# y00njaekim/CMU-11785-IDL-1.58bit-ASR

Hardware: AMD Instinct MI355X
Metric: mel-frames/sec (Conformer-S 1.58-bit train step) (higher is better)
Workload: dtype fp32; 1 GPU; conformer-s-1.58bit-train-step; global_batch=32, execution=hip-graph, per_gpu_batch=32, frames=1000, d_model=144, blocks=16, d_ff=576, heads=4, vocab=5004, parallelism=dp1, passes=teacher 2-bit + student 1-bit + SP, conv_pointwise=fp32 (reference)

## Files before the change

cmu-11785-idl-1.58bit-asr_amd/csrc/capi.hip:

```cpp
#include <algorithm>
#include <vector>

#include "../../include/onebit_hip.h"
#include "ob_launch.h"
#include <stdint.h>

using namespace ob;

namespace {

constexpr int kAbiVersion = 4;

inline hipStream_t as_stream(void* s) { return reinterpret_cast<hipStream_t>(s); }

inline bool aligned4(const void* p) { return (reinterpret_cast<uintptr_t>(p) & 3) == 0; }

inline int check_bits(int bits) { return (bits == 1 || bits == 2) ? OB_OK : OB_ERR_BITWIDTH; }

inline int launched() {
  const hipError_t e = hipGetLastError();
  return e == hipSuccess ? OB_OK : OB_ERR_HIP;
}

inline size_t align_up(size_t x) { return (x + 255) & ~size_t(255); }

struct DwWorkspace {
  size_t part, part_db, apart, total;
};

DwWorkspace dw_layout(int64_t P, int64_t M, int64_t N, int64_t K, int64_t G = 1) {
  const DwPlan p = plan_dw_passes(P, M, G * N, K);
  DwWorkspace w;
  w.part = align_up(sizeof(float) * (size_t)p.chunks * (size_t)N * (size_t)K);
  w.part_db = align_up(sizeof(float) * (size_t)p.chunks * (size_t)N);
  const int64_t napart = std::max<int64_t>(ste_reduce_blocks(N * K + N),
                                           p.tiles_n * p.tiles_k * p.chunks);
  w.apart = align_up(16 + sizeof(float) * (size_t)napart);
  w.total = w.part + w.part_db + w.apart;
  return w;
}

}

extern "C" {

int ob_abi_version(void) { return kAbiVersion; }

const char* ob_status_string(int status) {
  switch (status) {
    case OB_OK: return "ok";
    case OB_ERR_NULL: return "null pointer argument";
    case OB_ERR_SHAPE: return "invalid shape";
    case OB_ERR_BITWIDTH: return "bitwidth must be one of {1,2,32}";
    case OB_ERR_WORKSPACE: return "workspace too small";
    case OB_ERR_ALIGN: return "pointer not 4-byte aligned";
    case OB_ERR_HIP: return "HIP launch error";
    default: return "unknown status";
  }
}

int ob_quant_pack(const float* W, const float* alpha, int alpha_raw, int bits, int64_t N,
                  int64_t K, uint32_t* codes, uint32_t* codes_t, void* stream) {
  if (int st = check_bits(bits)) return st;
  if (N < 0 || K < 0) return OB_ERR_SHAPE;
// ... 310 lines not shown
      (nln > 1 && (!a16(ln_y1) || !a16(ln_w1) || !a16(ln_b1))) || !aligned4(bias) ||
      !aligned4(lens) || !aligned4(ln_mean0) || !aligned4(ln_rstd0) || !aligned4(ln_mean1) ||
      !aligned4(ln_rstd1))
    return OB_ERR_ALIGN;
  TgemmEpi ep{};
  ep.mode = kEpiResidual;
  ep.R = R;
  ep.rscale = rscale;
  ep.lens = reinterpret_cast<const int*>(lens);
  ep.T = (int)T;
  ep.p_drop = p_drop;
  ep.rng = rng;
  ep.rng_off = (uint64_t)rng_offset;
  ep.nln = nln;
  ep.lng[0] = ln_w0;
  ep.lnb[0] = ln_b0;
  ep.lneps[0] = eps0;
  ep.lny[0] = ln_y0;
  ep.lnmean[0] = ln_mean0;
  ep.lnrstd[0] = ln_rstd0;
  ep.lng[1] = ln_w1;
  ep.lnb[1] = ln_b1;
  ep.lneps[1] = eps1;
  ep.lny[1] = ln_y1;
  ep.lnmean[1] = ln_mean1;
  ep.lnrstd[1] = ln_rstd1;
  launch_ternary_gemm_passes(X, (int)P, M, K, codes2, pass_bits ? codes1 : codes2,
                             reinterpret_cast<const int*>(pass_bits), N, alpha, alpha_raw, bias, Y,
                             as_stream(stream), &ep);
  return launched();
}

int ob_bitlinear_bwd_dx_swish_drop(const float* dY, int64_t P, int64_t M, int64_t N,
                                   const uint32_t* codes2_t, const uint32_t* codes1_t,
                                   const int32_t* pass_bits, const float* alpha, int alpha_raw,
                                   int64_t K, const float* pre, float p_drop, const uint64_t* rng,
                                   int64_t rng_offset, float* dPre, void* stream) {
  if (int st = fused_gemm_check(dY, P, M, N, codes2_t, codes1_t, pass_bits, alpha, K, dPre, p_drop,
                                rng))
    return st;
  if (M * K > 0 && !pre) return OB_ERR_NULL;
  if (!aligned4(pre)) return OB_ERR_ALIGN;
  TgemmEpi ep{};
  ep.mode = kEpiSwishDropBwd;
  ep.R = pre;
  ep.p_drop = p_drop;
  ep.rng = rng;
  ep.rng_off = (uint64_t)rng_offset;
  launch_ternary_gemm_passes(dY, (int)P, M, N, codes2_t, pass_bits ? codes1_t : codes2_t,
                             reinterpret_cast<const int*>(pass_bits), K, alpha, alpha_raw, nullptr,
                             dPre, as_stream(stream), &ep);
  return launched();
}

int ob_drop_scale_bwd(const float* dOut, int64_t rows, int64_t N, float rscale, float p_drop,
                      const uint64_t* rng, int64_t rng_offset, const int32_t* lens, int64_t T,
                      float* dY, void* stream) {
  if (rows < 0 || N < 0 || !(p_drop >= 0.0f && p_drop < 1.0f)) return OB_ERR_SHAPE;
  if (lens && (T < 1 || T > 0x7fffffff || rows % T)) return OB_ERR_SHAPE;
  if ((rows * N > 0 && (!dOut || !dY)) || (p_drop > 0.0f && !rng)) return OB_ERR_NULL;
  if ((reinterpret_cast<uintptr_t>(dOut) & 15) || (reinterpret_cast<uintptr_t>(dY) & 15) ||
      !aligned4(lens))
    return OB_ERR_ALIGN;
  launch_drop_scale_bwd(dOut, rows, N, rscale, p_drop, rng, (uint64_t)rng_offset,
                        reinterpret_cast<const int*>(lens), (int)T, dY, as_stream(stream));
  return launched();
}

int ob_residual_drop_fwd(const float* R, const float* Y, int64_t rows, int64_t N, float rscale,
                         float p_drop, const uint64_t* rng, int64_t rng_offset,
                         const int32_t* lens, int64_t T, float* out, void* stream) {
  if (rows < 0 || N < 0 || !(p_drop >= 0.0f && p_drop < 1.0f)) return OB_ERR_SHAPE;
  if (lens && (T < 1 || T > 0x7fffffff || rows % T)) return OB_ERR_SHAPE;
  if ((rows * N > 0 && (!R || !Y || !out)) || (p_drop > 0.0f && !rng)) return OB_ERR_NULL;
  if (!aligned4(R) || !aligned4(Y) || !aligned4(out) || !aligned4(lens)) return OB_ERR_ALIGN;
  launch_residual_drop_fwd(R, Y, rows, N, rscale, p_drop, rng, (uint64_t)rng_offset,
                           reinterpret_cast<const int*>(lens), (int)T, out, as_stream(stream));
  return launched();
}

int ob_bias_relu_fwd(float* y, const float* bias, int64_t B, int64_t C, int64_t hw,
                     void* stream) {
  if (B < 0 || C < 0 || hw < 0) return OB_ERR_SHAPE;
  if (B * C * hw > 0 && (!y || !bias)) return OB_ERR_NULL;
  if (!aligned4(y) || !aligned4(bias)) return OB_ERR_ALIGN;
  if (hw % 4 == 0 && (reinterpret_cast<uintptr_t>(y) & 15)) return OB_ERR_ALIGN;
  launch_bias_relu_fwd(y, bias, B, C, hw, as_stream(stream));
  return launched();
}

size_t ob_relu_bias_bwd_workspace(int64_t B, int64_t C) {
  return (B < 0 || C < 0) ? 0 : relu_bias_bwd_workspace(B, C);
}

int ob_relu_bias_bwd(const float* g, const float* y, int64_t B, int64_t C, int64_t hw,
                     float* gout, float* dbias, void* ws, size_t ws_bytes, void* stream) {
  if (B < 0 || C < 0 || hw < 0 || B * C > 0x7fffffff) return OB_ERR_SHAPE;
  if (B * C * hw > 0 && (!g || !y || !gout)) return OB_ERR_NULL;
  if (B * C > 0 && !ws) return OB_ERR_NULL;
  if (ws_bytes < relu_bias_bwd_workspace(B, C)) return OB_ERR_WORKSPACE;
  if (!aligned4(g) || !aligned4(y) || !aligned4(gout) || !aligned4(dbias)) return OB_ERR_ALIGN;
  launch_relu_bias_bwd(g, y, B, C, hw, gout, dbias, ws, as_stream(stream));
  return launched();
}

size_t ob_colsum_workspace(int64_t N) { return N < 0 ? 0 : colsum_workspace(N); }
// ... 1177 lines not shown
```

cmu-11785-idl-1.58bit-asr_amd/csrc/ob_launch.h:

```cpp
#pragma once

#include <hip/hip_runtime.h>
#include <stddef.h>
#include <stdint.h>

#include "../../include/onebit_hip.h"

namespace ob {

inline int64_t ceil_div(int64_t a, int64_t b) { return (a + b - 1) / b; }

void launch_quant_pack(const float* W, const float* alpha, int alpha_raw, int bits,
                       const int* bits_dev, int64_t N, int64_t K, uint32_t* codes,
                       uint32_t* codes_t, hipStream_t s);
int64_t quant_pack_item_blocks(int64_t N, int64_t K);
int64_t quant_pack_item_blocks16(int64_t N, int64_t K);
void launch_quant_pack_group(const ob_pack_item* items_dev, int n_items, int64_t total_blocks,
                             hipStream_t s);
void launch_quant_dequant(const float* W, const float* alpha, int alpha_raw, int bits, int64_t n,
                          float* W_hat, hipStream_t s);

int64_t ste_reduce_blocks(int64_t total);
void launch_ste_reduce(const float* part, int chunks, int64_t nk, const float* part_db,
                       int64_t n_db, const float* W, const float* alpha, int alpha_raw, int bits,
                       const int* bits_dev, float* dW, float* db, float* apart, uint32_t* ticket,
                       float* dalpha, hipStream_t s);
constexpr int kMaxPasses = 4;
void launch_ste_reduce_passes(const float* part, int P, int cpp, int64_t nk, const float* part_db,
                              int64_t n_db, const float* W, const float* alpha, int alpha_raw,
                              const int* pass_bits, float* dW, float* db, float* apart,
                              uint32_t* ticket, float* dalpha, hipStream_t s);

bool launch_ternary_gemm_signacc(const float* A, int64_t M, int64_t K, const uint32_t* codes,
                                 int64_t N, const float* alpha, int alpha_raw, const float* bias,
                                 float* C, hipStream_t s);
void launch_ternary_gemm(const float* A, int64_t M, int64_t K, const uint32_t* codes, int64_t N,
                         const float* alpha, int alpha_raw, const float* bias, float* C,
                         hipStream_t s);

struct TgemmEpi;
void launch_ternary_gemm_passes(const float* A, int P, int64_t M, int64_t K,
                                const uint32_t* codes, const uint32_t* codes1,
                                const int* pass_bits, int64_t N, const float* alpha,
                                int alpha_raw, const float* bias, float* C, hipStream_t s,
                                const TgemmEpi* ep = nullptr);
bool launch_ternary_gemm_passes_group(const float* A, int P, int64_t M, int64_t K, int G,
                                      const uint32_t* const* codes,
                                      const uint32_t* const* codes1, const int* pass_bits,
                                      int64_t N, const float* const* alpha, int alpha_raw,
                                      const float* const* bias, float* const* C, hipStream_t s);
bool launch_ternary_dx_sum(int G, const float* const* dY, int P, int64_t M, int64_t N,
                           const uint32_t* const* codes_t, const uint32_t* const* codes_t1,
                           const int* pass_bits, const float* const* alpha, int alpha_raw,
                           int64_t K, float* dX, hipStream_t s);

enum { kEpiNone = 0, kEpiSwishDrop = 1, kEpiResidual = 2, kEpiSwishDropBwd = 3 };
struct TgemmEpi {
  int mode;
  const float* R;
  float* C2;
  float rscale;
  const int* lens;
  int T;
  float p_drop;
  const uint64_t* rng;
  uint64_t rng_off;
  int nln;
  const float* lng[2];
  const float* lnb[2];
  float lneps[2];
  float* lny[2];
  float* lnmean[2];
  float* lnrstd[2];
};
bool ternary_residual_ln_supported(int64_t K, int64_t N, int alpha_raw);

void launch_residual_drop_fwd(const float* R, const float* Y, int64_t rows, int64_t N,
                              float rscale, float p_drop, const uint64_t* rng, uint64_t rng_off,
                              const int* lens, int T, float* out, hipStream_t s);

void launch_bias_relu_fwd(float* y, const float* bias, int64_t B, int64_t C, int64_t hw,
                          hipStream_t s);
size_t relu_bias_bwd_workspace(int64_t B, int64_t C);
void launch_relu_bias_bwd(const float* g, const float* y, int64_t B, int64_t C, int64_t hw,
                          float* gout, float* dbias, void* ws, hipStream_t s);
void launch_zero_words(void* p, int64_t n_words, hipStream_t s);
size_t colsum_workspace(int64_t N);
void launch_colsum(const float* x, int64_t rows, int64_t N, float* out, void* ws, hipStream_t s);

bool decattn_supported(int64_t Lq, int64_t Lk, int64_t dh);
void launch_decattn_fwd(const float* q, int64_t sq, const float* k, int64_t sk, const float* v,
                        int64_t sv, const uint8_t* kmask, int causal, int64_t B, int64_t H,
                        int64_t Lq, int64_t Lk, int64_t dh, float p_drop, const uint64_t* rng,
                        uint64_t rng_off, float* probs, float* ctx, hipStream_t s);
void launch_decattn_bwd(const float* dctx, const float* ctxo, const float* q, int64_t sq,
                        const float* k, int64_t sk, const float* v, int64_t sv, int64_t B, int64_t H, int64_t Lq, int64_t Lk,
                        int64_t dh, float p_drop, float* probs, float* dq, int64_t gq,
                        float* dk, int64_t gk, float* dv, int64_t gv, hipStream_t s);
// ... 293 lines not shown
```

cmu-11785-idl-1.58bit-asr_amd/csrc/tgemm.hip:

```cpp
#include <cstdlib>

#include "ob_drop.h"
#include "ob_fp.h"
#include "ob_ln.h"
#include "ob_launch.h"
#include "ob_quant.h"

namespace ob {

namespace {

typedef float f32x4 __attribute__((ext_vector_type(4)));
typedef __bf16 bf16x8 __attribute__((ext_vector_type(8)));
typedef uint32_t u32x4 __attribute__((ext_vector_type(4)));

constexpr int kThreads = 256;
constexpr int kRows = 64;
constexpr size_t kMaxLds = 80 * 1024;
constexpr int kTargetBlocks = 512;
constexpr int kTargetBlocksLongK = 256;
constexpr int kByteWaves = 8;
constexpr int kBPad = 16;
constexpr int kBytePad = 8;

__device__ __forceinline__ void code_bytes(uint32_t word, u32x4& out) {
#pragma unroll
  for (int q = 0; q < 4; ++q) {
    uint32_t x = (word >> (8 * q)) & 0xFFu;
    x = (x | (x << 6) | (x << 12) | (x << 18)) & 0x03030303u;
    const uint32_t lo = x & 0x01010101u, hi = x & 0x02020202u;
    out[q] = ((lo << 6) - lo) | (hi << 6);
  }
}

__device__ __forceinline__ bf16x8 bytes_bf16x8(uint32_t d0, uint32_t d1) {
  u32x4 o;
  o[0] = __builtin_amdgcn_perm(d1, d0, 0x010C000Cu);
  o[1] = __builtin_amdgcn_perm(d1, d0, 0x030C020Cu);
  o[2] = __builtin_amdgcn_perm(d1, d0, 0x050C040Cu);
  o[3] = __builtin_amdgcn_perm(d1, d0, 0x070C060Cu);
  return __builtin_bit_cast(bf16x8, o);
}

#ifdef OB_TGEMM_STAMPS
__device__ uint64_t g_tg_stamps[32768];
__device__ uint64_t g_tg_rt[16384];
#define TG_DECL                                                              \
  uint64_t tg_t = __builtin_amdgcn_s_memtime(), tg_rt0 = __builtin_amdgcn_s_memrealtime(), \
           tg_acc[4] = {0, 0, 0, 0};
#define TG_STAMP(k)                                       \
  do {                                                    \
    const uint64_t tg_n = __builtin_amdgcn_s_memtime();   \
// ... 568 lines not shown
            } else {
              epi_store4<EPI>(ep, dkey, C + orow * N + col, rowbase + orow, col, N, y, rvalid[it],
                              rpre[it]);
            }
          }
        }
        asm volatile("s_waitcnt lgkmcnt(0)" ::: "memory");
        __builtin_amdgcn_sched_barrier(0);
      }
      TG_STAMP(2);
      continue;
    }
    if constexpr (!VEC_EPI) {

    constexpr bool kHasR = EPI == kEpiResidual || EPI == kEpiSwishDropBwd;
    constexpr int kPre = 2;
    float rv[NT][4];
    auto load_r = [&](int t) {
      const int col = min(n0 + 16 * t + r, N - 1);
#pragma unroll
      for (int reg = 0; reg < 4; ++reg) {
        const int64_t orow = min(m0 + 4 * g + reg, M - 1);
        rv[t][reg] = ep.R[(rowbase + orow) * N + col];
      }
    };
    if constexpr (kHasR) {
#pragma unroll
      for (int t = 0; t < kPre && t < NT; ++t) load_r(t);
    }
#pragma unroll
    for (int t = 0; t < NT; ++t) {
      if constexpr (kHasR) {
        if (t + kPre < NT) load_r(t + kPre);
        __builtin_amdgcn_sched_barrier(0);
      }
      const int col = n0 + 16 * t + r;
      if (col >= N) continue;
#pragma unroll
      for (int reg = 0; reg < 4; ++reg) {
        const int64_t orow = m0 + 4 * g + reg;
        if (orow >= M) continue;
        const float y = fmaf(a_eff, acc[t][reg], bcol[t]);
        if constexpr (EPI == kEpiNone) {
          C[orow * N + col] = y;
          if (EPI == kEpiSwishDrop) ep.C2[(rowbase + orow) * N + col] = y;
        } else {
          epi_store<EPI>(ep, dkey, C + orow * N + col, rowbase + orow, col, N, y, rv[t][reg]);
        }
      }
      if constexpr (EPI != kEpiNone) __builtin_amdgcn_sched_barrier(0);
    }
    TG_STAMP(2);
    }
  }
  TG_WRITE
}

constexpr int kF32NT = 3;

__global__ __launch_bounds__(kThreads) void tgemm_f32_kernel(
    const float* __restrict__ A, int64_t M, int64_t K, const uint32_t* __restrict__ codes,
    int64_t KW, int64_t N, const float* __restrict__ alpha, int alpha_raw,
    const float* __restrict__ bias, float* __restrict__ C, const uint32_t* __restrict__ codes1,
    const int* __restrict__ pass_bits, EpiArgs ep) {
  const int64_t rowbase = pass_bits ? (int64_t)blockIdx.z * M : 0;
  if (pass_bits) {
    const int p = blockIdx.z;
    if (pass_bits[p] == 1) codes = codes1;
    A += (int64_t)p * M * K;
    C += (int64_t)p * M * N;
  }
  const int lane = threadIdx.x & 63;
  const int wave = threadIdx.x >> 6;
  const int r = lane & 15;
  const int g = lane >> 4;
  const int64_t m0 = (int64_t)blockIdx.x * kRows + wave * 16;
  const int64_t n0 = (int64_t)blockIdx.y * (16 * kF32NT);
  const int64_t row = m0 + r < M ? m0 + r : M - 1;
  const float* arow = A + row * K;
  f32x4 acc[kF32NT];
#pragma unroll
  for (int t = 0; t < kF32NT; ++t) acc[t] = f32x4{0.f, 0.f, 0.f, 0.f};
  for (int64_t kc = 0; kc < K; kc += 16) {
    float xa[4];
#pragma unroll
    for (int e = 0; e < 4; ++e) {
      const int64_t k = kc + 4 * g + e;
      xa[e] = arow[k < K ? k : K - 1];
    }
#pragma unroll
    for (int t = 0; t < kF32NT; ++t) {
      const int64_t n = n0 + 16 * t + r;
      if (alpha_raw >= 2) {
        const uint16_t* Wb = reinterpret_cast<const uint16_t*>(codes);
#pragma unroll
        for (int e = 0; e < 4; ++e) {
          const int64_t k = kc + 4 * g + e;
          const float w = (n < N && k < K) ? __uint_as_float((uint32_t)Wb[n * K + k] << 16) : 0.0f;
          acc[t] = __builtin_amdgcn_mfma_f32_16x16x4f32(xa[e], w, acc[t], 0, 0, 0);
        }
        continue;
      }
      const uint32_t word = codes[(n < N ? n : N - 1) * KW + (kc >> 4)];
      const uint32_t byte = (n < N) ? (word >> (8 * g)) : 0u;
#pragma unroll
      for (int e = 0; e < 4; ++e)
// ... 73 lines not shown
  const size_t lds = epi_stage_off(NT, kpad, byte) +
                     (byte && ep.mode == kEpiResidual
                          ? (size_t)wv * 16 * (16 * NT + 4) * sizeof(float) + 4 * 16 * NT * sizeof(float)
                          : epi_stage_bytes(NT, wv));
  const int KW = (int)ceil_div(K, 16);
  const bool vec = (N % 4 == 0) && aligned16(C) && (ep.mode != kEpiSwishDrop || aligned16(ep.C2)) &&
                   ((ep.mode != kEpiResidual && ep.mode != kEpiSwishDropBwd) || aligned16(ep.R));
#define OB_TGEMM_E(NCH, E)                                                                     \
  if (vec)                                                                                    \
    hipLaunchKernelGGL((tgemm_bf16x3_kernel<NT, NCH, E, true>), grid, dim3(kThreads), lds, s,  \
                       A, M, (int)K, codes, KW, (int)N, n_ct, n16, rgroups, alpha, alpha_raw,  \
                       bias, C, codes1, pass_bits, ep);                                         \
  else                                                                                        \
    hipLaunchKernelGGL((tgemm_bf16x3_kernel<NT, NCH, E, false>), grid, dim3(kThreads), lds, s, \
                       A, M, (int)K, codes, KW, (int)N, n_ct, n16, rgroups, alpha, alpha_raw,  \
                       bias, C, codes1, pass_bits, ep)
  if constexpr (NT == 9) {
    if (byte) {
#define OB_TGEMM_B(E)                                                                            \
  if (vec)                                                                                      \
    hipLaunchKernelGGL((tgemm_bf16x3_kernel<9, 18, E, true, true, 1, kByteWaves>), grid,         \
                       dim3(64 * kByteWaves), lds, s,                                            \
                       A, M, (int)K, codes, KW, (int)N, n_ct, n16, rgroups, alpha, alpha_raw,    \
                       bias, C, codes1, pass_bits, ep);                                           \
  else                                                                                          \
    hipLaunchKernelGGL((tgemm_bf16x3_kernel<9, 18, E, false, true, 1, kByteWaves>), grid,        \
                       dim3(64 * kByteWaves), lds,                                               \
                       s, A, M, (int)K, codes, KW, (int)N, n_ct, n16, rgroups, alpha, alpha_raw, \
                       bias, C, codes1, pass_bits, ep)
      if (ep.mode == kEpiResidual) OB_TGEMM_B(kEpiResidual);
      else OB_TGEMM_B(kEpiNone);
#undef OB_TGEMM_B
      return;
    }
  }
#define OB_TGEMM(NCH)                                                   \
  switch (ep.mode) {                                                    \
    case kEpiSwishDrop: OB_TGEMM_E(NCH, kEpiSwishDrop); break;          \
    case kEpiResidual: OB_TGEMM_E(NCH, kEpiResidual); break;            \
    case kEpiSwishDropBwd: OB_TGEMM_E(NCH, kEpiSwishDropBwd); break;    \
    default: OB_TGEMM_E(NCH, kEpiNone); break;                          \
  }
  switch ((K + 31) / 32) {
    case 2: OB_TGEMM(2); break;
    case 5: OB_TGEMM(5); break;
    case 8: OB_TGEMM(8); break;
    case 18: OB_TGEMM(18); break;
    default: OB_TGEMM(0); break;
  }
#undef OB_TGEMM
#undef OB_TGEMM_E
}

}

void launch_ternary_gemm_passes(const float* A, int P, int64_t M, int64_t K,
                                const uint32_t* codes, const uint32_t* codes1,
                                const int* pass_bits, int64_t N, const float* alpha,
                                int alpha_raw, const float* bias, float* C, hipStream_t s,
                                const TgemmEpi* epi) {
  if (M == 0 || N == 0 || P == 0) return;
  EpiArgs ep{};
  ep.glayers = 1;
  ep.mode = kEpiNone;
  if (epi && epi->mode != kEpiNone) {
    ep.mode = epi->mode;
    ep.R = epi->R;
    ep.C2 = epi->C2;
    ep.rscale = epi->rscale;
    ep.lens = epi->lens;
    ep.T = epi->T > 0 ? epi->T : 1;
    ep.dc = make_drop(epi->p_drop);
    ep.rng = epi->rng;
    ep.rng_off = epi->rng_off;
    ep.nln = epi->nln;
    for (int i = 0; i < 2; ++i) {
      ep.lng[i] = epi->lng[i];
      ep.lnb[i] = epi->lnb[i];
      ep.lneps[i] = epi->lneps[i];
      ep.lny[i] = epi->lny[i];
      ep.lnmean[i] = epi->lnmean[i];
      ep.lnrstd[i] = epi->lnrstd[i];
    }
  }
  const bool vec = (K % 4 == 0) && K >= 4 && ((reinterpret_cast<uintptr_t>(A) & 15) == 0);
  const int nt = vec && !use_f32_gemm() ? pick_nt(N, K, ep.mode) : 0;
  if (nt > 0 && (K + 31) / 32 == 18 && N % 144 == 0 && alpha_raw < 2 &&
      (ep.mode == kEpiNone || ep.mode == kEpiResidual)) {
    launch_bf16x3<9>(A, M, K, codes, N, alpha, alpha_raw, bias, C, codes1, pass_bits, P, ep, s, true);
    return;
  }
#define OB_NT(V)                                                                            \
  case V:                                                                                   \
    launch_bf16x3<V>(A, M, K, codes, N, alpha, alpha_raw, bias, C, codes1, pass_bits, P, ep, s); \
    return;
  switch (nt) {
    OB_NT(12)
    OB_NT(9)
    OB_NT(6)
    OB_NT(4)
    OB_NT(3)
    OB_NT(2)
    OB_NT(1)
    default: break;
  }
#undef OB_NT
  const dim3 grid((unsigned)ceil_div(M, kRows), (unsigned)ceil_div(N, 16 * kF32NT), (unsigned)P);
  hipLaunchKernelGGL(tgemm_f32_kernel, grid, dim3(kThreads), 0, s, A, M, K, codes,
                     ceil_div(K, 16), N, alpha, alpha_raw, bias, C, codes1, pass_bits, ep);
}

bool launch_ternary_gemm_passes_group(const float* A, int P, int64_t M, int64_t K, int G,
                                      const uint32_t* const* codes,
                                      const uint32_t* const* codes1, const int* pass_bits,
                                      int64_t N, const float* const* alpha, int alpha_raw,
                                      const float* const* bias, float* const* C, hipStream_t s) {
  if (G < 1 || G > 3) return false;
  const bool vec = (K % 4 == 0) && K >= 4 && ((reinterpret_cast<uintptr_t>(A) & 15) == 0);
  const int nt = vec && !use_f32_gemm() ? pick_nt(N, K, kEpiNone) : 0;
  if (M == 0 || N == 0 || P == 0) return true;
  bool al = (N % 4 == 0);
  for (int i = 0; i < G; ++i) al = al && aligned16(C[i]);
  if (nt == 0 || N % (16 * nt) != 0 || !al) {
    for (int i = 0; i < G; ++i)
      launch_ternary_gemm_passes(A, P, M, K, codes[i], codes1[i], pass_bits, N, alpha[i],
                                 alpha_raw, bias[i], C[i], s);
    return true;
  }
  EpiArgs ep{};
  ep.glayers = G;
  ep.mode = kEpiNone;
  for (int i = 0; i < G; ++i) {
    ep.gcodes[i] = codes[i];
    ep.gcodes1[i] = codes1[i];
    ep.galpha[i] = alpha[i];
    ep.gbias[i] = bias[i];
    ep.gC[i] = C[i];
  }
#define OB_NTG(V)                                                                                \
  case V:                                                                                        \
    launch_bf16x3<V>(A, M, K, codes[0], N, alpha[0], alpha_raw, bias[0], C[0], codes1[0],       \
                     pass_bits, P, ep, s);                                                       \
    return true;
  switch (nt) {
// ... 66 lines not shown
```

cmu-11785-idl-1.58bit-asr_amd/onebit_asr/_lib.py:

```python
from __future__ import annotations

import ctypes
import os
from pathlib import Path

import torch

LIB_NAME = "libonebit_hip.so"
LIB_PATH = Path(os.environ.get("ONEBIT_HIP_LIB") or Path(__file__).with_name(LIB_NAME))

OB_OK = 0
OB_ERR_SHAPE = -2
OB_ERR_BITWIDTH = -3

_c_f = ctypes.c_void_p
_i64 = ctypes.c_int64
_int = ctypes.c_int
_sz = ctypes.c_size_t
_f32 = ctypes.c_float
_f64 = ctypes.c_double

SIGNATURES = {
    "ob_abi_version": (_int, []),
    "ob_source_digest": (ctypes.c_char_p, []),
    "ob_status_string": (ctypes.c_char_p, [_int]),
    "ob_quant_pack": (_int, [_c_f, _c_f, _int, _int, _i64, _i64, _c_f, _c_f, _c_f]),
    "ob_quant_pack_item_blocks": (_i64, [_i64, _i64]),
    "ob_quant_pack_group": (_int, [_c_f, _int, _i64, _c_f]),
    "ob_weight_bf16_item_blocks": (_i64, [_i64, _i64]),
    "ob_bitlinear_fwd_swish_drop": (
        _int, [_c_f, _i64, _i64, _i64, _c_f, _c_f, _c_f, _c_f, _int, _c_f, _i64, _f32, _c_f, _i64,
               _c_f, _c_f, _c_f]),
    "ob_bitlinear_fwd_residual": (
        _int, [_c_f, _i64, _i64, _i64, _c_f, _c_f, _c_f, _c_f, _int, _c_f, _i64, _c_f, _f32, _f32,
               _c_f, _i64, _c_f, _i64, _c_f, _c_f]),
    "ob_bitlinear_bwd_dx_swish_drop": (
        _int, [_c_f, _i64, _i64, _i64, _c_f, _c_f, _c_f, _c_f, _int, _i64, _c_f, _f32, _c_f, _i64,
               _c_f, _c_f]),
    "ob_drop_scale_bwd": (_int, [_c_f, _i64, _i64, _f32, _f32, _c_f, _i64, _c_f, _i64, _c_f, _c_f]),
    "ob_residual_drop_fwd": (
        _int, [_c_f, _c_f, _i64, _i64, _f32, _f32, _c_f, _i64, _c_f, _i64, _c_f, _c_f]),
    "ob_convmod_workspace": (_sz, [_i64, _i64, _i64, _i64, _i64]),
    "ob_convmod_fwd": (
        _int, [_c_f, _c_f, _c_f, _c_f, _c_f, _i64, _i64, _i64, _i64, _i64, _f32, _c_f, _c_f, _c_f,
               _c_f, _c_f, _sz, _c_f]),
    "ob_convmod_bwd": (
        _int, [_c_f, _c_f, _c_f, _c_f, _c_f, _c_f, _c_f, _c_f, _i64, _i64, _i64, _i64, _i64, _c_f,
               _c_f, _c_f, _c_f, _c_f, _c_f, _sz, _c_f]),
    "ob_convmod_bwd_defer": (
        _int, [_c_f, _c_f, _c_f, _c_f, _c_f, _c_f, _c_f, _c_f, _i64, _i64, _i64, _i64, _i64, _c_f,
               _c_f, _c_f, _c_f, _c_f, _c_f, _sz, _c_f, _i64, _c_f, _c_f]),
    "ob_decattn_supported": (_int, [_i64, _i64, _i64]),
    "ob_decattn_fwd": (_int, [_c_f, _i64, _c_f, _i64, _c_f, _i64, _c_f, _i64, _i64, _i64, _i64,
                              _i64, _i64, _f32, _c_f, _i64, _c_f, _c_f, _c_f]),
    "ob_decattn_bwd": (_int, [_c_f, _c_f, _c_f, _i64, _c_f, _i64, _c_f, _i64, _i64, _i64, _i64, _i64,
                              _i64, _f32, _c_f, _c_f, _i64, _c_f, _i64, _c_f, _i64, _c_f]),
    "ob_cm_wgrad_entry_bytes": (_sz, []),
    "ob_cm_wgrad_table": (_int, [_c_f, _i64, _i64, _c_f]),
    "ob_bias_relu_fwd": (_int, [_c_f, _c_f, _i64, _i64, _i64, _c_f]),
    "ob_relu_bias_bwd_workspace": (_sz, [_i64, _i64]),
    "ob_relu_bias_bwd": (_int, [_c_f, _c_f, _i64, _i64, _i64, _c_f, _c_f, _c_f, _sz, _c_f]),
    "ob_colsum_workspace": (_sz, [_i64]),
    "ob_colsum": (_int, [_c_f, _i64, _i64, _c_f, _c_f, _sz, _c_f]),
    "ob_dense_supported": (_int, [_i64, _i64]),
    "ob_silu_fast_monotone_check": (_int, [ctypes.c_uint32, ctypes.c_uint32, _c_f, _c_f]),
    "ob_dense_gemm_residual_drop": (_int, [_c_f, _i64, _i64, _c_f, _c_f, _i64, _c_f, _f32, _c_f,
                                            _i64, _c_f, _c_f]),
    "ob_dense_gemm": (_int, [_c_f, _i64, _i64, _c_f, _int, _c_f, _i64, _c_f, _c_f]),
    "ob_dense_dw_workspace": (_sz, [_i64, _i64, _i64]),
    "ob_dense_dw": (_int, [_c_f, _c_f, _i64, _i64, _i64, _c_f, _c_f, _c_f, _sz, _c_f]),
    "ob_subsample_image_bytes": (_sz, [_i64]),
    "ob_subsample_pack": (_int, [_c_f, _i64, _c_f, _c_f]),
    "ob_subsample_fwd": (_int, [_c_f, _i64, _i64, _i64, _i64, _c_f, _c_f, _c_f, _c_f, _c_f,
                                _c_f, _c_f]),
    "ob_subsample_bwd_workspace": (_sz, [_i64, _i64, _i64, _i64]),
    "ob_subsample_bwd": (_int, [_c_f, _c_f, _c_f, _c_f, _c_f, _c_f, _i64, _i64, _i64, _i64, _c_f,
                                _c_f, _c_f, _c_f, _c_f, _c_f, _sz, _c_f]),
    "ob_ctc_loss_fwd_groups": (
        _int, [_c_f, _c_f, _c_f, _c_f, _i64, _i64, _i64, _i64, _i64, _int, _c_f, _c_f, _sz, _c_f]),
    "ob_ctc_loss_bwd_groups": (
        _int, [_c_f, _c_f, _c_f, _c_f, _i64, _i64, _i64, _i64, _i64, _int, _c_f, _c_f, _c_f, _sz,
               _c_f]),
    "ob_ctc_logits_workspace": (_sz, [_i64, _i64, _i64]),
    "ob_ctc_loss_logits_fwd_groups": (
        _int, [_c_f, _c_f, _c_f, _c_f, _i64, _i64, _i64, _i64, _i64, _int, _c_f, _c_f, _sz, _c_f]),
    "ob_ctc_loss_logits_bwd_groups": (
        _int, [_c_f, _c_f, _c_f, _c_f, _i64, _i64, _i64, _i64, _i64, _int, _c_f, _c_f, _c_f, _sz,
               _c_f]),
    "ob_att_kl_workspace": (_sz, [_i64, _i64]),
    "ob_att_kl_loss_fwd": (
        _int, [_c_f, _c_f, _c_f, _i64, _i64, _i64, _int, _f32, _c_f, _c_f, _c_f, _sz, _c_f]),
# ... 72 lines not shown
    "ob_dw_grouped": (_int, [_c_f, _i64, _c_f, _sz, _c_f, _sz, _c_f]),
    "ob_dense_dw_defer": (_int, [_c_f, _c_f, _i64, _i64, _i64, _c_f, _c_f, _c_f, _sz, _c_f, _i64,
                                 _i64, _c_f, _c_f]),
    "ob_layernorm_bwd_workspace": (_sz, [_i64, _i64]),
    "ob_layernorm_bwd": (
        _int, [_c_f, _c_f, _c_f, _c_f, _c_f, _i64, _i64, _c_f, _c_f, _c_f, _c_f, _sz, _c_f]),
    "ob_layernorm_bwd_res": (
        _int, [_c_f, _c_f, _c_f, _c_f, _c_f, _i64, _i64, _c_f, _c_f, _c_f, _c_f, _c_f, _sz, _c_f]),
    "ob_layernorm_bwd_ex": (
        _int, [_c_f, _c_f, _c_f, _c_f, _c_f, _i64, _i64, _c_f, _c_f, _c_f, _c_f, _c_f, _sz, _c_f,
               _f32, _f32, _c_f, _i64, _c_f, _i64, _c_f]),
    "ob_act_absmax_workspace": (_sz, [_i64]),
    "ob_act_absmax": (_int, [_c_f, _i64, _i64, _c_f, _c_f, _sz, _c_f]),
    "ob_act_dequant_i8": (_int, [_c_f, _i64, _i64, _c_f, _c_f, _c_f]),
    "ob_bitlinear_fwd_i8": (
        _int, [_c_f, _i64, _i64, _i64, _c_f, _c_f, _c_f, _c_f, _int, _c_f, _c_f, _i64, _c_f, _c_f]),
    "ob_bitlinear_fwd_i8_epi": (
        _int, [_c_f, _i64, _i64, _i64, _c_f, _c_f, _c_f, _c_f, _int, _c_f, _c_f, _i64, _int, _c_f,
               _f32, _c_f, _i64, _c_f, _c_f, _c_f]),
    "ob_bitlinear_fwd_passes_group": (
        _int, [_i64, _c_f, _i64, _i64, _i64, _c_f, _c_f, _c_f, _c_f, _int, _c_f, _i64, _c_f, _c_f]),
    "ob_bitlinear_fwd_i8q": (
        _int, [_c_f, _i64, _i64, _i64, _c_f, _c_f, _c_f, _c_f, _int, _c_f, _c_f, _i64, _int, _c_f,
               _f32, _c_f, _i64, _c_f, _c_f, _c_f]),
    "ob_bitlinear_bwd_dx_passes": (
        _int, [_c_f, _i64, _i64, _i64, _c_f, _c_f, _c_f, _c_f, _int, _i64, _c_f, _c_f]),
    "ob_bitlinear_bwd_dw_passes_workspace": (_sz, [_i64, _i64, _i64, _i64]),
    "ob_bitlinear_bwd_dw_passes": (
        _int, [_c_f, _c_f, _i64, _i64, _i64, _i64, _c_f, _c_f, _int, _c_f, _c_f, _c_f, _c_f, _c_f,
               _sz, _c_f]),
    "ob_bitlinear_bwd_dw_passes_group_workspace": (_sz, [_i64, _i64, _i64, _i64, _i64]),
    "ob_bitlinear_bwd_dw_passes_group": (
        _int, [_i64, _c_f, _c_f, _i64, _i64, _i64, _i64, _c_f, _c_f, _int, _c_f, _c_f, _c_f, _c_f,
               _c_f, _sz, _c_f]),
    "ob_relattn_fwd": (
        _int, [_c_f, _c_f, _c_f, _c_f, _c_f, _c_f, _c_f, _i64, _i64, _i64, _i64, _i64, _f32, _c_f,
               _i64, _c_f, _c_f, _c_f, _c_f]),
    "ob_relattn_saved_elems": (_i64, [_i64, _i64, _i64, _i64]),
    "ob_relattn_probs_elems": (_i64, [_i64, _i64, _i64]),
    "ob_relattn_bwd_workspace": (_sz, [_i64, _i64, _i64, _i64]),
    "ob_relattn_bwd": (
        _int, [_c_f, _c_f, _c_f, _c_f, _c_f, _c_f, _c_f, _c_f, _c_f, _i64, _i64, _i64, _i64, _i64,
               _f32, _c_f, _i64, _c_f, _i64, _c_f, _c_f, _c_f, _c_f, _c_f, _c_f, _c_f, _sz, _c_f]),
    "ob_relattn_set_bwd_mode": (_int, [_int]),
    "ob_relattn_dropout_mask": (_int, [_i64, _i64, _f32, _c_f, _i64, _c_f, _c_f]),
    "ob_embedding_bwd": (_int, [_c_f, _i64, _c_f, _i64, _i64, _i64, _c_f, _c_f]),
    "ob_adamw_plan": (_i64, [_c_f, _i64, _c_f]),
    "ob_adamw_workspace": (_sz, [_i64]),
    "ob_adamw_clip_step": (
        _int, [_c_f, _i64, _c_f, _i64, _c_f, _c_f, _f32, _f64, _f64, _f64, _f64, _f64, _c_f, _c_f,
               _sz, _c_f]),
}

ABI_VERSION = 4

_lib = None


class OneBitHipError(RuntimeError):
    pass


def load() -> ctypes.CDLL:
    global _lib
    if _lib is not None:
        return _lib
    if not LIB_PATH.is_file():
        raise OneBitHipError(
            f"{LIB_PATH} is missing: build it with `make -C cmu-11785-idl-1.58bit-asr_amd/csrc` "
            "(or __graft_entry__.build()); there is no CPU fallback for the BitLinear path"
        )
    lib = ctypes.CDLL(str(LIB_PATH))
    for name, (res, args) in SIGNATURES.items():
        fn = getattr(lib, name)
        fn.restype = res
        fn.argtypes = args
    if lib.ob_abi_version() != ABI_VERSION:
        raise OneBitHipError(f"ABI mismatch: library {lib.ob_abi_version()} != {ABI_VERSION}")
    check_digest(lib)
    _lib = lib
    return lib


def check_digest(lib, expected: str | None = None) -> None:
    if expected is None:
        if os.environ.get("ONEBIT_HIP_LIB"):
            return
        if not _sources_present():
            import warnings

            warnings.warn(f"{LIB_PATH.name}: no csrc/ sources beside it; build digest not checked")
            return
        expected = source_digest()
    got = lib.ob_source_digest().decode()
    if got != expected:
        raise OneBitHipError(
            f"{LIB_PATH.name} was built from other sources (digest {got[:12]} != {expected[:12]} "
            "of csrc/ and include/): rebuild with `make -C cmu-11785-idl-1.58bit-asr_amd/csrc`")


def _sources_present() -> bool:
    csrc = Path(__file__).resolve().parents[1] / "csrc"
    return csrc.is_dir() and any(csrc.glob("*.hip"))


def ptr_array(ptrs):
    return (ctypes.c_void_p * len(ptrs))(*[p or None for p in ptrs])
# ... 24 lines not shown
```

include/onebit_hip.h:

```cpp
#ifndef ONEBIT_HIP_H_
#define ONEBIT_HIP_H_

#include <stddef.h>
#include <stdint.h>

#ifdef __cplusplus
extern "C" {
#endif

#define OB_API __attribute__((visibility("default")))

enum {
  OB_OK = 0,
  OB_ERR_NULL = -1,
  OB_ERR_SHAPE = -2,
  OB_ERR_BITWIDTH = -3,
  OB_ERR_WORKSPACE = -4,
  OB_ERR_ALIGN = -5,
  OB_ERR_HIP = -6
};

OB_API int ob_abi_version(void);
OB_API const char* ob_source_digest(void);
OB_API const char* ob_status_string(int status);
// ... 289 lines not shown
OB_API size_t ob_layernorm_bwd_pair_workspace(int64_t rows, int64_t d);
OB_API int ob_layernorm_bwd_pair(const float* dy, const float* y1, const float* g2,
                                 const float* mean2, const float* rstd2, const float* gres,
                                 const float* x, const float* g1, const float* mean1,
                                 const float* rstd1, int64_t rows, int64_t d, float* dx,
                                 float* dg2, float* db2, float* dg1, float* db1, void* ws,
                                 size_t ws_bytes, float* dy2, float rscale, float p_drop,
                                 const uint64_t* rng, int64_t rng_offset, const int32_t* lens,
                                 int64_t T, void* table, int64_t slot2, int64_t slot1,
                                 void* stream);
OB_API size_t ob_ln_param_entry_bytes(void);
OB_API int ob_ln_param_table(const void* table, int64_t n, int64_t dmax, void* stream);

OB_API int ob_ctc_greedy_decode(const float* logits, const int64_t* lens, int64_t B, int64_t T,
                                int64_t V, int blank, int32_t* ids, int32_t* out,
                                int32_t* out_len, void* stream);

OB_API size_t ob_ctc_beam_search_workspace(int64_t B, int64_t T, int64_t V, int beam, int top_k);
OB_API int ob_ctc_beam_search(const float* logits, const int64_t* lens, int64_t B, int64_t T,
                              int64_t V, int blank, int beam, int top_k, void* ws,
                              size_t ws_bytes, int32_t* out, int32_t* out_len, double* score,
                              void* stream);
OB_API int ob_ctc_beam_search_stage(const float* logits, const int64_t* lens, int64_t B,
                                    int64_t T, int64_t V, int blank, int beam, int top_k,
                                    int stage, void* ws, size_t ws_bytes, int32_t* out,
                                    int32_t* out_len, double* score, void* stream);

OB_API int ob_bitlinear_fwd_swish_drop(const float* X, int64_t P, int64_t M, int64_t K,
                                       const uint32_t* codes2, const uint32_t* codes1,
                                       const int32_t* pass_bits, const float* alpha,
                                       int alpha_raw, const float* bias, int64_t N, float p_drop,
                                       const uint64_t* rng, int64_t rng_offset, float* Y_pre,
                                       float* Y_act, void* stream);
OB_API int ob_bitlinear_fwd_residual(const float* X, int64_t P, int64_t M, int64_t K,
                                     const uint32_t* codes2, const uint32_t* codes1,
                                     const int32_t* pass_bits, const float* alpha, int alpha_raw,
                                     const float* bias, int64_t N, const float* R, float rscale,
                                     float p_drop, const uint64_t* rng, int64_t rng_offset,
                                     const int32_t* lens, int64_t T, float* Y, void* stream);
OB_API int ob_bitlinear_fwd_residual_ln(
    const float* X, int64_t P, int64_t M, int64_t K, const uint32_t* codes2,
    const uint32_t* codes1, const int32_t* pass_bits, const float* alpha, int alpha_raw,
    const float* bias, int64_t N, const float* R, float rscale, float p_drop, const uint64_t* rng,
    int64_t rng_offset, const int32_t* lens, int64_t T, float* Y, int nln, const float* ln_w0,
    const float* ln_b0, float eps0, float* ln_y0, float* ln_mean0, float* ln_rstd0,
    const float* ln_w1, const float* ln_b1, float eps1, float* ln_y1, float* ln_mean1,
    float* ln_rstd1, void* stream);
OB_API int ob_bitlinear_bwd_dx_swish_drop(const float* dY, int64_t P, int64_t M, int64_t N,
                                          const uint32_t* codes2_t, const uint32_t* codes1_t,
                                          const int32_t* pass_bits, const float* alpha,
                                          int alpha_raw, int64_t K, const float* pre,
                                          float p_drop, const uint64_t* rng, int64_t rng_offset,
                                          float* dPre, void* stream);
OB_API int ob_drop_scale_bwd(const float* dOut, int64_t rows, int64_t N, float rscale,
                             float p_drop, const uint64_t* rng, int64_t rng_offset,
                             const int32_t* lens, int64_t T, float* dY, void* stream);

OB_API int ob_residual_drop_fwd(const float* R, const float* Y, int64_t rows, int64_t N,
                                float rscale, float p_drop, const uint64_t* rng,
                                int64_t rng_offset, const int32_t* lens, int64_t T, float* out,
                                void* stream);

OB_API int ob_bias_relu_fwd(float* y, const float* bias, int64_t B, int64_t C, int64_t hw,
                            void* stream);
OB_API size_t ob_relu_bias_bwd_workspace(int64_t B, int64_t C);
OB_API int ob_relu_bias_bwd(const float* g, const float* y, int64_t B, int64_t C, int64_t hw,
                            float* gout, float* dbias, void* ws, size_t ws_bytes, void* stream);
OB_API size_t ob_colsum_workspace(int64_t N);
OB_API int ob_colsum(const float* x, int64_t rows, int64_t N, float* out, void* ws,
                     size_t ws_bytes, void* stream);

OB_API int ob_silu_fast_monotone_check(uint32_t lo_bits, uint32_t hi_bits, uint32_t* bad,
                                       void* stream);
OB_API int ob_dense_supported(int64_t K, int64_t N);
OB_API int ob_dense_gemm(const float* X, int64_t M, int64_t K, const float* W, int w_trans,
                         const float* bias, int64_t N, float* Y, void* stream);
OB_API int ob_dense_gemm_residual_drop(const float* X, int64_t M, int64_t K, const float* W,
                                       const float* bias, int64_t N, const float* R,
                                       float p_drop, const int64_t* rng, int64_t rng_offset,
                                       float* Y, void* stream);
OB_API size_t ob_dense_dw_workspace(int64_t M, int64_t N, int64_t K);
OB_API int ob_dense_dw(const float* dY, const float* X, int64_t M, int64_t N, int64_t K,
                       float* dW, float* db, void* ws, size_t ws_bytes, void* stream);
OB_API int ob_dense_dw_defer(const float* dY, const float* X, int64_t M, int64_t N, int64_t K,
                             float* dW, float* db, void* ws, size_t ws_bytes, void* table,
                             int64_t slot, int64_t start, int64_t* n_blocks, void* stream);

OB_API size_t ob_convmod_workspace(int64_t P, int64_t Bt, int64_t T, int64_t C, int64_t K);
OB_API int ob_convmod_fwd(const float* u, const float* w_dw, const float* b_dw,
                          const float* gamma, const float* beta, int64_t P, int64_t Bt,
                          int64_t T, int64_t C, int64_t K, float eps, float* z, float* g,
                          float* stats, float* v, void* ws, size_t ws_bytes, void* stream);
OB_API int ob_convmod_bwd(const float* dv, const float* u, const float* z, const float* g,
                          const float* stats, const float* w_dw, const float* gamma,
                          const float* beta, int64_t P, int64_t Bt, int64_t T, int64_t C,
                          int64_t K, float* du, float* dw_dw, float* db_dw, float* dgamma,
                          float* dbeta, void* ws, size_t ws_bytes, void* stream);
OB_API int ob_convmod_bwd_defer(const float* dv, const float* u, const float* z, const float* g,
                                const float* stats, const float* w_dw, const float* gamma,
                                const float* beta, int64_t P, int64_t Bt, int64_t T, int64_t C,
                                int64_t K, float* du, float* dw_dw, float* db_dw, float* dgamma,
                                float* dbeta, void* ws, size_t ws_bytes, void* table, int64_t slot,
                                int64_t* deferred, void* stream);
OB_API size_t ob_cm_wgrad_entry_bytes(void);
OB_API int ob_cm_wgrad_table(const void* table, int64_t n, int64_t nmax, void* stream);

// ... 18 lines not shown
```

Baseline: 1.414 million mel-frames/s.

## Add wide-N ternary GEMM kernel for swish-dropout FFN GEMMs with full-N LDS image

Adds a specialized ternary GEMM kernel for N=576, K≤160 (the FFN up-projection and its swish backward). Each persistent block decodes the whole weight code matrix once into LDS and then sweeps row tiles, with 8 waves split into older/younger halves, bf16x3 MFMA accumulation, and a staged vectorized epilogue through LDS. It is enabled by default through an env var or API toggle. The aim is to avoid repeated per-tile code decode and scattered stores, at the cost of heavy LDS use (~100KB) and occupancy of one block per CU.

Result: no change. 1.424 million mel-frames/s, median of 6 (+0.7%).

```diff
diff --git a/cmu-11785-idl-1.58bit-asr_amd/csrc/capi.hip b/cmu-11785-idl-1.58bit-asr_amd/csrc/capi.hip
--- a/cmu-11785-idl-1.58bit-asr_amd/csrc/capi.hip
+++ b/cmu-11785-idl-1.58bit-asr_amd/csrc/capi.hip
@@ -9,7 +9,7 @@
 
 namespace {
 
-constexpr int kAbiVersion = 4;
+constexpr int kAbiVersion = 5;
 
 inline hipStream_t as_stream(void* s) { return reinterpret_cast<hipStream_t>(s); }
 
@@ -426,6 +426,8 @@
                              dPre, as_stream(stream), &ep);
   return launched();
 }
+
+int ob_tgemm_set_wide(int mode) { return tgemm_set_wide(mode); }
 
 int ob_drop_scale_bwd(const float* dOut, int64_t rows, int64_t N, float rscale, float p_drop,
                       const uint64_t* rng, int64_t rng_offset, const int32_t* lens, int64_t T,
diff --git a/cmu-11785-idl-1.58bit-asr_amd/csrc/ob_launch.h b/cmu-11785-idl-1.58bit-asr_amd/csrc/ob_launch.h
--- a/cmu-11785-idl-1.58bit-asr_amd/csrc/ob_launch.h
+++ b/cmu-11785-idl-1.58bit-asr_amd/csrc/ob_launch.h
@@ -44,6 +44,7 @@
                                 const int* pass_bits, int64_t N, const float* alpha,
                                 int alpha_raw, const float* bias, float* C, hipStream_t s,
                                 const TgemmEpi* ep = nullptr);
+int tgemm_set_wide(int on);
 bool launch_ternary_gemm_passes_group(const float* A, int P, int64_t M, int64_t K, int G,
                                       const uint32_t* const* codes,
                                       const uint32_t* const* codes1, const int* pass_bits,
diff --git a/cmu-11785-idl-1.58bit-asr_amd/csrc/tgemm.hip b/cmu-11785-idl-1.58bit-asr_amd/csrc/tgemm.hip
--- a/cmu-11785-idl-1.58bit-asr_amd/csrc/tgemm.hip
+++ b/cmu-11785-idl-1.58bit-asr_amd/csrc/tgemm.hip
@@ -1,3 +1,4 @@
+#include <atomic>
 #include <cstdlib>
 
 #include "ob_drop.h"
@@ -672,6 +673,196 @@
     }
     TG_STAMP(2);
     }
+  }
+  TG_WRITE
+}
+
+constexpr int kWideN = 576;
+constexpr int kWideNch = 5;
+constexpr int kWidePitch = 176;
+constexpr int kWideWaves = 8;
+constexpr int kWideBlocks = 256;
+constexpr int kWideOlder16 = 9;
+constexpr int kWideNT = 4;
+constexpr int kWideLd = 16 * kWideNT;
+constexpr size_t kWideImgBytes = (size_t)kWideN * kWidePitch;
+constexpr size_t kWideLds =
+    kWideImgBytes + kWideN * sizeof(float) + (size_t)kWideWaves * 16 * kWideLd * sizeof(float);
+static_assert(kWideLds <= 160 * 1024, "wide form: one block's LDS");
+
+__device__ __forceinline__ void code_bytes_lut(uint32_t word, u32x4& out) {
+#pragma unroll
+  for (int q = 0; q < 4; ++q) {
+    uint32_t x = (word >> (8 * q)) & 0xFFu;
+    x = (x | (x << 6) | (x << 12) | (x << 18)) & 0x03030303u;
+    out[q] = __builtin_amdgcn_perm(0u, 0xBF803F00u, x);
+  }
+}
+
+template <int EPI, int WV>
+__global__ __launch_bounds__(64 * WV, 1) void tgemm_wide_kernel(
+    const float* __restrict__ A, int64_t M, int K, const uint32_t* __restrict__ codes, int KW,
+    int n16, int rgroups, const float* __restrict__ alpha, int alpha_raw,
+    const float* __restrict__ bias, float* __restrict__ C, const uint32_t* __restrict__ codes1,
+    const int* __restrict__ pass_bits, EpiArgs ep) {
+  static_assert(EPI == kEpiSwishDrop || EPI == kEpiSwishDropBwd, "wide form: swish epilogues");
+  TG_DECL
+  constexpr int kThr = 64 * WV, N = kWideN, NCH = kWideNch, NT = kWideNT, NG = N / (16 * NT);
+  constexpr int stride = kWidePitch, kwp = 2 * NCH, nwords = N * kwp;
+  constexpr bool kHasR = EPI == kEpiSwishDropBwd;
+  select_pass(A, C, codes, codes1, pass_bits, M, K, N);
+  const int64_t rowbase = pass_bits ? (int64_t)blockIdx.y * M : 0;
+  extern __shared__ __attribute__((aligned(16))) char smem[];
+  float* biasS = reinterpret_cast<float*>(smem + kWideImgBytes);
+  const int lane = threadIdx.x & 63;
+  const int wave = __builtin_amdgcn_readfirstlane(threadIdx.x >> 6);
+  const int r = lane & 15;
+  const int g = lane >> 4;
+  const int kg = 8 * g;
+  float* stg = biasS + N + wave * 16 * kWideLd;
+  const int rg = blockIdx.x;
+  const int s0 = (int)((int64_t)rg * n16 / rgroups), s1 = (int)((int64_t)(rg + 1) * n16 / rgroups);
+  auto arow_of = [&](int j) {
+    const int64_t row = (int64_t)16 * j + r < M ? (int64_t)16 * j + r : M - 1;
+    return A + row * (int64_t)K;
+  };
+  static_assert(WV == 8, "wide form: two waves a SIMD");
+  const int U = (s1 - s0) * NG;
+  const int q = wave & 3, p0 = U * q / 4, p1 = U * (q + 1) / 4;
+  const int older = ((p1 - p0) * kWideOlder16 + 8) / 16;
+  int u = wave < 4 ? p0 : p0 + older;
+  const int uend = wave < 4 ? p0 + older : p1;
+
+  constexpr int kWpt = (nwords + kThr - 1) / kThr;
+  uint32_t wv[kWpt];
+#pragma unroll
+  for (int i = 0; i < kWpt; ++i) {
+    const int idx = min((int)threadIdx.x + i * kThr, nwords - 1);
+    const int nl = idx / kwp, w = idx - nl * kwp;
+    wv[i] = codes[nl * KW + (w < KW ? w : KW - 1)];
+  }
+  f32x4 buf[NCH][2];
+  {
+    const int j0 = s0 + u / NG < n16 ? s0 + u / NG : n16 - 1;
+    const float* a0 = arow_of(j0);
+#pragma unroll
+    for (int c = 0; c < NCH; ++c) load8(a0, 32 * c + kg, K, buf[c][0], buf[c][1]);
+  }
+  constexpr int kBpt = (N + kThr - 1) / kThr;
+  float bv[kBpt];
+#pragma unroll
+  for (int i = 0; i < kBpt; ++i) {
+    const int c = min((int)threadIdx.x + i * kThr, N - 1);
+    bv[i] = bias ? bias[c] : 0.0f;
+  }
+  const float a_eff = 2.0f * effective_alpha(alpha, alpha_raw);
+  const uint32_t dkey = ep.dc.on ? drop_key(ep.rng[0], ep.rng[1] + ep.rng_off) : 0u;
+  __builtin_amdgcn_sched_barrier(0);
+#pragma unroll
+  for (int i = 0; i < kWpt; ++i) {
+    const int idx = threadIdx.x + i * kThr;
+    const int nl = idx / kwp, w = idx - nl * kwp;
+    u32x4 b4;
+    code_bytes_lut(w < KW ? wv[i] : 0u, b4);
+    if (idx < nwords) *reinterpret_cast<u32x4*>(smem + nl * stride + 16 * w) = b4;
+  }
+#pragma unroll
+  for (int i = 0; i < kBpt; ++i)
+    if ((int)threadIdx.x + i * kThr < N) biasS[threadIdx.x + i * kThr] = bv[i];
+  __syncthreads();
+  TG_STAMP(0);
+
+  const unsigned char* brow8 = reinterpret_cast<const unsigned char*>(smem) + r * stride + kg;
+  typedef uint32_t u32x2 __attribute__((ext_vector_type(2)));
+  constexpr int kQ = 16;
+
+  while (u < uend) {
+    const int sl = u / NG, ga = u - sl * NG;
+    const int gb = ga + (uend - u) < NG ? ga + (uend - u) : NG;
+    const int unext = u + (gb - ga);
+    const int64_t m0 = (int64_t)16 * (s0 + sl);
+    bf16x8 hi[NCH], mid[NCH], lo[NCH];
+#pragma unroll
+    for (int c = 0; c < NCH; ++c) split3(buf[c][0], buf[c][1], hi[c], mid[c], lo[c]);
+    __builtin_amdgcn_sched_barrier(0);
+    if (unext < uend) {
+      const float* an = arow_of(s0 + unext / NG);
+#pragma unroll
+      for (int c = 0; c < NCH; ++c) load8(an, 32 * c + kg, K, buf[c][0], buf[c][1]);
+    }
+    __builtin_amdgcn_sched_barrier(0);
+
+    u32x2 bb[NCH][NT];
+    float bcol[NT];
+    auto read_b = [&](int gi) {
+      const unsigned char* bg = brow8 + gi * (16 * NT) * stride;
+#pragma unroll
+      for (int c = 0; c < NCH; ++c)
+#pragma unroll
+        for (int t = 0; t < NT; ++t)
+          bb[c][t] = *reinterpret_cast<const u32x2*>(bg + t * 16 * stride + 32 * c);
+#pragma unroll
+      for (int t = 0; t < NT; ++t) bcol[t] = biasS[gi * (16 * NT) + 16 * t + r];
+    };
+    read_b(ga);
+#pragma unroll 1
+    for (int gi = ga; gi < gb; ++gi) {
+      const int n0 = gi * (16 * NT);
+      f32x4 rpre[NT];
+      if constexpr (kHasR) {
+#pragma unroll
+        for (int it = 0; it < NT; ++it) {
+          const int idx = it * 64 + lane, row = idx / kQ, c4 = idx - row * kQ;
+          const int64_t orow = m0 + row < M ? m0 + row : M - 1;
+          rpre[it] = *reinterpret_cast<const f32x4*>(ep.R + (rowbase + orow) * N + n0 + 4 * c4);
+        }
+      }
+      __builtin_amdgcn_sched_barrier(0);
+      f32x4 acc[NT];
+#pragma unroll
+      for (int t = 0; t < NT; ++t) acc[t] = f32x4{0.f, 0.f, 0.f, 0.f};
+#pragma unroll
+      for (int c = 0; c < NCH; ++c) {
+#pragma unroll
+        for (int t = 0; t < NT; ++t) {
+          const bf16x8 b = bytes_bf16x8(bb[c][t][0], bb[c][t][1]);
+          acc[t] = mfma_bf16(lo[c], b, acc[t]);
+          acc[t] = mfma_bf16(mid[c], b, acc[t]);
+          acc[t] = mfma_bf16(hi[c], b, acc[t]);
+        }
+      }
+#pragma unroll
+      for (int t = 0; t < NT; ++t)
+#pragma unroll
+        for (int reg = 0; reg < 4; ++reg) acc[t][reg] = fmaf(a_eff, acc[t][reg], bcol[t]);
+      __builtin_amdgcn_sched_barrier(0);
+      TG_STAMP(1);
+      read_b(gi + 1 < gb ? gi + 1 : gi);
+      __builtin_amdgcn_sched_barrier(0);
+#pragma unroll
+      for (int t = 0; t < NT; ++t)
+#pragma unroll
+        for (int reg = 0; reg < 4; ++reg) stg[(4 * g + reg) * kWideLd + 16 * t + r] = acc[t][reg];
+      asm volatile("s_waitcnt lgkmcnt(0)" ::: "memory");
+      __builtin_amdgcn_sched_barrier(0);
+#pragma unroll
+      for (int it = 0; it < NT; ++it) {
+        const int idx = it * 64 + lane, row = idx / kQ, c4 = idx - row * kQ;
+        const int64_t orow = m0 + row;
+        const int col = n0 + 4 * c4;
+        const f32x4 y = *reinterpret_cast<const f32x4*>(stg + row * kWideLd + 4 * c4);
+        if (orow < M)
+          epi_store4<EPI>(ep, dkey, C + orow * N + col, rowbase + orow, col, N, y, true,
+                          kHasR ? rpre[it] : y);
+      }
+      asm volatile("s_waitcnt lgkmcnt(0)" ::: "memory");
+      __builtin_amdgcn_sched_barrier(0);
+      TG_STAMP(2);
+    }
+#ifdef OB_TGEMM_STAMPS
+    ++tg_acc[3];
+#endif
+    u = unext;
   }
   TG_WRITE
 }
@@ -851,6 +1042,43 @@
 #undef OB_TGEMM_E
 }
 
+void launch_wide(const float* A, int64_t M, int64_t K, const uint32_t* codes, const float* alpha,
+                 int alpha_raw, const float* bias, float* C, const uint32_t* codes1,
+                 const int* pass_bits, int P, const EpiArgs& ep, hipStream_t s) {
+  const int n16 = (int)ceil_div(M, 16);
+  int rgroups = kWideBlocks / P;
+  if (rgroups > n16) rgroups = n16;
+  if (rgroups < 1) rgroups = 1;
+  const dim3 grid((unsigned)rgroups, (unsigned)P);
+  const int KW = (int)ceil_div(K, 16);
+  if (ep.mode == kEpiSwishDrop)
+    hipLaunchKernelGGL((tgemm_wide_kernel<kEpiSwishDrop, kWideWaves>), grid, dim3(64 * kWideWaves),
+                       kWideLds, s, A, M, (int)K, codes, KW, n16, rgroups, alpha, alpha_raw, bias,
+                       C, codes1, pass_bits, ep);
+  else
+    hipLaunchKernelGGL((tgemm_wide_kernel<kEpiSwishDropBwd, kWideWaves>), grid,
+                       dim3(64 * kWideWaves), kWideLds, s, A, M, (int)K, codes, KW, n16, rgroups,
+                       alpha, alpha_raw, bias, C, codes1, pass_bits, ep);
+}
+
+std::atomic<int> g_wide{-1};
+bool wide_selected() {
+  int m = g_wide.load(std::memory_order_relaxed);
+  if (m < 0) {
+    const char* e = getenv("OB_TGEMM_WIDE");
+    int want = (e != nullptr && e[0] == '0') ? 0 : 1;
+    g_wide.compare_exchange_strong(m, want);
+    m = g_wide.load(std::memory_order_relaxed);
+  }
+  return m == 1;
+}
+
+}
+
+int tgemm_set_wide(int on) {
+  const int prev = wide_selected() ? 1 : 0;
+  if (on == 0 || on == 1) g_wide.store(on, std::memory_order_relaxed);
+  return prev;
 }
 
 void launch_ternary_gemm_passes(const float* A, int P, int64_t M, int64_t K,
@@ -889,6 +1117,13 @@
     launch_bf16x3<9>(A, M, K, codes, N, alpha, alpha_raw, bias, C, codes1, pass_bits, P, ep, s, true);
     return;
   }
+  if (nt > 0 && (K + 31) / 32 == kWideNch && N == kWideN && alpha_raw < 2 && aligned16(C) &&
+      ((ep.mode == kEpiSwishDrop && aligned16(ep.C2)) ||
+       (ep.mode == kEpiSwishDropBwd && aligned16(ep.R))) &&
+      wide_selected()) {
+    launch_wide(A, M, K, codes, alpha, alpha_raw, bias, C, codes1, pass_bits, P, ep, s);
+    return;
+  }
 #define OB_NT(V)                                                                            \
   case V:                                                                                   \
     launch_bf16x3<V>(A, M, K, codes, N, alpha, alpha_raw, bias, C, codes1, pass_bits, P, ep, s); \
diff --git a/cmu-11785-idl-1.58bit-asr_amd/onebit_asr/_lib.py b/cmu-11785-idl-1.58bit-asr_amd/onebit_asr/_lib.py
--- a/cmu-11785-idl-1.58bit-asr_amd/onebit_asr/_lib.py
+++ b/cmu-11785-idl-1.58bit-asr_amd/onebit_asr/_lib.py
@@ -37,6 +37,7 @@
     "ob_bitlinear_bwd_dx_swish_drop": (
         _int, [_c_f, _i64, _i64, _i64, _c_f, _c_f, _c_f, _c_f, _int, _i64, _c_f, _f32, _c_f, _i64,
                _c_f, _c_f]),
+    "ob_tgemm_set_wide": (_int, [_int]),
     "ob_drop_scale_bwd": (_int, [_c_f, _i64, _i64, _f32, _f32, _c_f, _i64, _c_f, _i64, _c_f, _c_f]),
     "ob_residual_drop_fwd": (
         _int, [_c_f, _c_f, _i64, _i64, _f32, _f32, _c_f, _i64, _c_f, _i64, _c_f, _c_f]),
@@ -215,7 +216,7 @@
                _sz, _c_f]),
 }
 
-ABI_VERSION = 4
+ABI_VERSION = 5
 
 _lib = None
 
diff --git a/include/onebit_hip.h b/include/onebit_hip.h
--- a/include/onebit_hip.h
+++ b/include/onebit_hip.h
@@ -365,6 +365,7 @@
                                           int alpha_raw, int64_t K, const float* pre,
                                           float p_drop, const uint64_t* rng, int64_t rng_offset,
                                           float* dPre, void* stream);
+OB_API int ob_tgemm_set_wide(int mode);
 OB_API int ob_drop_scale_bwd(const float* dOut, int64_t rows, int64_t N, float rscale,
                              float p_drop, const uint64_t* rng, int64_t rng_offset,
                              const int32_t* lens, int64_t T, float* dY, void* stream);
```
